# jgrodzki/radix_sort

Hardware: AMD Instinct MI355X
Metric: Gkeys/sec (u64) (higher is better)
Workload: dtype u64

## Files before the change

radix_sort_amd/csrc/rsx_small_kernel.hpp:

```cpp
#pragma once
#include "rsx_device.hpp"
#include "rsx_internal.hpp"

namespace rsx {

struct SmallArgs {
    const void* src;
    void* data;
    uint32_t n;
    uint32_t passes;
    uint32_t rank_atomic;
    uint32_t map_load;
    uint32_t map_store;
    DigitSpec spec[16];
    KeyXform xf;
    const uint32_t* top_tot;
    uint32_t cap;
    uint32_t no_skip;
    uint32_t group_shift;
    uint32_t key_offset, key_bytes;
    uint32_t* hint;
};

struct PassPlan {
    uint32_t first, end;
    uint32_t mask[8];
    uint32_t low[8];
    __device__ __forceinline__ void set_masks(const uint32_t key_offset, const uint32_t key_bytes) {
#pragma unroll
        for (int w = 0; w < 8; ++w) {
            uint32_t m = 0, l = 0;
#pragma unroll
            for (uint32_t b = 0; b < 4; ++b) {
                const uint32_t byte = 4u * (uint32_t)w + b;
                if (byte >= key_offset + first && byte < key_offset + key_bytes) m |= 0xFFu << (8u * b);
                if (byte >= key_offset && byte < key_offset + first) l |= 0xFFu << (8u * b);
            }
            mask[w] = m;
            low[w] = l;
        }
    }
};

#ifndef RSX_MEND_SLACK
#define RSX_MEND_SLACK 6u
#endif
__device__ __forceinline__ uint32_t first_digit_for(const uint32_t m, const uint32_t variable_bits, const uint32_t end) {
    const uint32_t lg = m <= 1u ? 0u : 32u - (uint32_t)__builtin_clz(m - 1u);
    const uint32_t need = 2u * lg > RSX_MEND_SLACK ? 2u * lg - RSX_MEND_SLACK : 0u;
    uint32_t first = variable_bits > need ? (variable_bits - need) >> 3 : 0u;
    if (first + 1u > end) first = end != 0u ? end - 1u : 0u;
    return first;
}

template <int ES>
struct WaveCnt {
    static constexpr bool HALF = false;
    using T = typename std::conditional<HALF, uint16_t, uint32_t>::type;
    static __device__ __forceinline__ void zero(T* my, uint32_t lane) {
        uint32_t* w = reinterpret_cast<uint32_t*>(my);
#pragma unroll
        for (int i = 0; i < (HALF ? 2 : 4); ++i) w[i * WAVE + lane] = 0;
    }
    static __device__ __forceinline__ uint32_t add_rtn(T* my, uint32_t d, uint32_t v) {
        if constexpr (HALF) {
            const uint32_t sh = (d & 1u) * 16u;
            return (atomicAdd(reinterpret_cast<uint32_t*>(my) + (d >> 1), v << sh) >> sh) & 0xFFFFu;
        } else {
            return atomicAdd(&my[d], v);
        }
    }
};
template <int ES, int KPT, int WG>
__host__ __device__ constexpr uint32_t cape() {
    constexpr uint32_t c = rsxh::bucket_cape(ES, KPT, WG);
    return c;
}
template <int ES, int KPT, int WG>
struct LdsTile {
    using C = typename WaveCnt<ES>::T;
    static_assert(sizeof(C) == rsxh::bucket_cnt_bytes(), "host and device agree on the wave counters");
    static constexpr int NWAVE = WG / WAVE;
    __host__ __device__ static constexpr size_t bytes() { return rsxh::lds_tile_bytes(ES, KPT, WG); }
    static __device__ __forceinline__ Elem<ES>* elems(unsigned char* smem) { return reinterpret_cast<Elem<ES>*>(smem); }
    static __device__ __forceinline__ C* cnt(unsigned char* smem) { return reinterpret_cast<C*>(smem + (size_t)cape<ES, KPT, WG>() * ES); }
    static __device__ __forceinline__ uint32_t* misc(unsigned char* smem) { return reinterpret_cast<uint32_t*>(cnt(smem) + NWAVE * RADIX); }
    static __device__ __forceinline__ uint32_t* flag(unsigned char* smem) { return misc(smem) + NWAVE; }
};

struct Slots { uint32_t kp, seg; };
template <int WG>
__device__ __forceinline__ Slots slots_of(const uint32_t n) {
    const uint32_t tid = threadIdx.x, lane = tid & 63u, wave = tid >> 6;
    const uint32_t kp = (n + WG - 1) / WG;
    return Slots{kp, wave * (WAVE * kp) + lane};
}
template <int ES, int KPT, int WG>
__device__ __forceinline__ void local_load(const SmallArgs& a, const Elem<ES>* __restrict__ src, const uint32_t n, Elem<ES> (&e)[KPT]) {
    const Slots sl = slots_of<WG>(n);
    const uint32_t kp = sl.kp, seg = sl.seg;
#pragma unroll
    for (int j = 0; j < KPT; ++j) {
        e[j] = Elem<ES>{};
        if ((uint32_t)j < kp) {
            const uint32_t p = seg + (uint32_t)j * WAVE;
            if (p < n) {
                e[j] = src[p];
                if (a.map_load) key_map<ES, false>(e[j], a.xf);
            }
        }
    }
}

template <int ES, int KPT, int WG>
__device__ __forceinline__ void local_passes(const SmallArgs& a, Elem<ES> (&e)[KPT], const uint32_t n, unsigned char* smem,
                                             const uint32_t first = 0, const uint32_t end = ~0u) {
    const uint32_t stop = end == ~0u ? a.passes : end;
    constexpr int NWAVE = WG / WAVE;
    using E = Elem<ES>;
    using C = WaveCnt<ES>;
    using Tile = LdsTile<ES, KPT, WG>;
    E* s_elems = Tile::elems(smem);
    typename C::T* s_cnt = Tile::cnt(smem);
    uint32_t* s_misc = Tile::misc(smem);
    const uint32_t tid = threadIdx.x, lane = tid & 63u, wave = tid >> 6;
    const Slots sl = slots_of<WG>(n);
    const uint32_t kp = sl.kp, seg = sl.seg;
    typename C::T* my = s_cnt + wave * RADIX;
    for (uint32_t pass = first; pass < stop; ++pass) {
        const DigitSpec spec = a.spec[pass];
        C::zero(my, lane);
        auto digit_of = [&](int j) -> uint32_t {
            return (seg + (uint32_t)j * WAVE >= n) ? 255u : elem_digit<ES, false>(e[j], spec);
        };
        uint32_t rk[KPT];
#pragma unroll
        for (int j = 0; j < KPT; ++j) {
            rk[j] = 0;
            if ((uint32_t)j < kp) {
                const uint32_t d = digit_of(j);
                if (a.rank_atomic) {
                    rk[j] = C::add_rtn(my, d, 1u);
                } else {
                    const uint64_t m = match_digit(d);
                    const uint32_t below = mbcnt64(m);
                    const uint32_t seen = my[d];
                    if (below == 0) (void)C::add_rtn(my, d, (uint32_t)__popcll(m));
                    rk[j] = seen + below;
                }
            }
        }
        __syncthreads();
        uint32_t tcount = 0, incl = 0;
        if (tid < RADIX) {
#pragma unroll
            for (int w = 0; w < NWAVE; ++w) tcount += s_cnt[w * RADIX + tid];
            incl = wave_incl_scan<true>(tcount);
            if (lane == 63) s_misc[wave] = incl;
        }
        __syncthreads();
        if (tid < RADIX) {
            uint32_t run = incl - tcount;
            for (uint32_t w = 0; w < wave; ++w) run += s_misc[w];
#pragma unroll
            for (int w = 0; w < NWAVE; ++w) {
                const uint32_t c = s_cnt[w * RADIX + tid];
                s_cnt[w * RADIX + tid] = (typename C::T)run;
                run += c;
            }
        }
        __syncthreads();
#pragma unroll
        for (int j = 0; j < KPT; ++j)
            if ((uint32_t)j < kp) {
                if constexpr (cape<ES, KPT, WG>() < (uint32_t)WG * KPT) {
                    if (seg + (uint32_t)j * WAVE < n) s_elems[(uint32_t)my[digit_of(j)] + rk[j]] = e[j];
                } else {
                    s_elems[(uint32_t)my[digit_of(j)] + rk[j]] = e[j];
                }
            }
        __syncthreads();
        if (pass + 1 < stop) {
#pragma unroll
            for (int j = 0; j < KPT; ++j)
                if ((uint32_t)j < kp) e[j] = s_elems[seg + (uint32_t)j * WAVE];
        }
    }
}

template <int ES, int KPT, int WG>
__device__ __forceinline__ void local_store(const SmallArgs& a, Elem<ES>* __restrict__ dst, const uint32_t n, unsigned char* smem) {
    const Elem<ES>* s_elems = reinterpret_cast<const Elem<ES>*>(smem);
    for (uint32_t i = threadIdx.x; i < n; i += WG) {
        Elem<ES> x = s_elems[i];
        if (a.map_store) key_map<ES, true>(x, a.xf);
        dst[i] = x;
    }
}

template <int ES, int KPT, int WG>
__device__ __forceinline__ void local_sort(const SmallArgs& a, const Elem<ES>* __restrict__ src, Elem<ES>* __restrict__ dst,
                                           const uint32_t n, unsigned char* smem) {
    Elem<ES> e[KPT];
    local_load<ES, KPT, WG>(a, src, n, e);
    local_passes<ES, KPT, WG>(a, e, n, smem);
    local_store<ES, KPT, WG>(a, dst, n, smem);
}

template <int ES, int KPT, int WG, typename DigitFn>
__device__ __forceinline__ void stream_pass(const SmallArgs& a, const Elem<ES>* __restrict__ src, Elem<ES>* __restrict__ dst, const uint32_t m,
                                            unsigned char* smem, DigitFn digit, const bool map_back, uint32_t& bin_start, uint32_t& bin_count) {
    constexpr int NWAVE = WG / WAVE;
    constexpr uint32_t CH = cape<ES, KPT, WG>();
    using E = Elem<ES>;
    using C = WaveCnt<ES>;
    using Tile = LdsTile<ES, KPT, WG>;
    E* s_elems = Tile::elems(smem);
    typename C::T* s_cnt = Tile::cnt(smem);
    uint32_t* s_misc = Tile::misc(smem);
    uint32_t* s_gbase = s_misc + NWAVE;
    uint32_t* s_dstart = s_gbase + RADIX;
    uint32_t* s_dcount = s_dstart + RADIX;
    const uint32_t tid = threadIdx.x, lane = tid & 63u, wave = tid >> 6;
    typename C::T* my = s_cnt + wave * RADIX;
    if (tid < RADIX) s_gbase[tid] = 0;
    __syncthreads();
    for (uint32_t i = tid; i < m; i += WG) atomicAdd(&s_gbase[digit(src[i])], 1u);
    __syncthreads();
    if (tid < RADIX) {
        const uint32_t c = s_gbase[tid];
        const uint32_t incl = wave_incl_scan<true>(c);
        if (lane == 63) s_misc[wave] = incl;
        s_dcount[tid] = incl - c;
        bin_count = c;
    }
    __syncthreads();
    if (tid < RADIX) {
        uint32_t b = s_dcount[tid];
        for (uint32_t w = 0; w < wave; ++w) b += s_misc[w];
        s_gbase[tid] = b;
        bin_start = b;
    }
    __syncthreads();
    for (uint32_t c0 = 0; c0 < m; c0 += CH) {
        const uint32_t n = m - c0 < CH ? m - c0 : CH;
        const Slots sl = slots_of<WG>(n);
        const uint32_t kp = sl.kp, seg = sl.seg;
        E e[KPT];
#pragma unroll
        for (int j = 0; j < KPT; ++j) {
            e[j] = E{};
            if ((uint32_t)j < kp) {
                const uint32_t p = seg + (uint32_t)j * WAVE;
                if (p < n) e[j] = src[c0 + p];
            }
        }
        C::zero(my, lane);
        auto digit_of = [&](int j) -> uint32_t { return (seg + (uint32_t)j * WAVE >= n) ? 255u : digit(e[j]); };
        uint32_t rk[KPT];
#pragma unroll
        for (int j = 0; j < KPT; ++j) {
            rk[j] = 0;
            if ((uint32_t)j < kp) {
                const uint32_t d = digit_of(j);
                const uint64_t mm = match_digit(d);
                const uint32_t below = mbcnt64(mm);
                const uint32_t seen = my[d];
                if (below == 0) (void)C::add_rtn(my, d, (uint32_t)__popcll(mm));
                rk[j] = seen + below;
            }
        }
        __syncthreads();
        uint32_t tcount = 0, incl = 0;
        if (tid < RADIX) {
#pragma unroll
            for (int w = 0; w < NWAVE; ++w) tcount += s_cnt[w * RADIX + tid];
            incl = wave_incl_scan<true>(tcount);
            if (lane == 63) s_misc[wave] = incl;
        }
        __syncthreads();
        if (tid < RADIX) {
            uint32_t run = incl - tcount;
            for (uint32_t w = 0; w < wave; ++w) run += s_misc[w];
            s_dstart[tid] = run;
            s_dcount[tid] = tid == RADIX - 1 ? tcount - (kp * WG - n) : tcount;
#pragma unroll
            for (int w = 0; w < NWAVE; ++w) {
                const uint32_t c = s_cnt[w * RADIX + tid];
                s_cnt[w * RADIX + tid] = (typename C::T)run;
                run += c;
            }
        }
        __syncthreads();
#pragma unroll
        for (int j = 0; j < KPT; ++j)
            if ((uint32_t)j < kp) {
                if constexpr (cape<ES, KPT, WG>() < (uint32_t)WG * KPT) {
                    if (seg + (uint32_t)j * WAVE < n) s_elems[(uint32_t)my[digit_of(j)] + rk[j]] = e[j];
                } else {
                    s_elems[(uint32_t)my[digit_of(j)] + rk[j]] = e[j];
                }
            }
        __syncthreads();
        for (uint32_t i = tid; i < n; i += WG) {
            E x = s_elems[i];
            const uint32_t d = digit(x);
            const uint32_t pos = s_gbase[d] + (i - s_dstart[d]);
            if (map_back) key_map<ES, true>(x, a.xf);
            dst[pos] = x;
        }
        __syncthreads();
        if (tid < RADIX) s_gbase[tid] += s_dcount[tid];
        __syncthreads();
    }
    __builtin_amdgcn_fence(__ATOMIC_RELEASE, "agent");
    __syncthreads();
    __builtin_amdgcn_fence(__ATOMIC_ACQUIRE, "agent");
}

template <int ES, int KPT, int WG>
__device__ void big_bucket_sort(const SmallArgs& a, Elem<ES>* buf0, Elem<ES>* buf1, const uint32_t m, unsigned char* smem) {
    using E = Elem<ES>;
    E* src = buf0;
    E* dst = buf1;
    for (uint32_t pass = 0; pass < a.passes; ++pass) {
        const DigitSpec spec = a.spec[pass];
        uint32_t bs = 0, bc = 0;
        stream_pass<ES, KPT, WG>(a, src, dst, m, smem, [&](const E& x) { return elem_digit<ES, false>(x, spec); },
                                 pass + 1 == a.passes && a.map_store != 0, bs, bc);
        E* t = src;
        src = dst;
        dst = t;
    }
}

#define RSX_B16_WAVES(WG) ((WG) >= 512 ? 4 : 3)
template <int ES>
__device__ __forceinline__ bool agree(const PassPlan& pp, const Elem<ES>& x, const Elem<ES>& y) {
    uint32_t diff = 0;
#pragma unroll
    for (int w = 0; w < ES / 4; ++w) diff |= (x.w[w] ^ y.w[w]) & pp.mask[w];
    return diff == 0;
}
constexpr uint32_t MEND_LIST = 192;
template <int ES, int KPT, int WG>
__device__ __forceinline__ uint32_t* mend_count(unsigned char* smem) {
    return reinterpret_cast<uint32_t*>(LdsTile<ES, KPT, WG>::cnt(smem));
}
template <int ES, int KPT, int WG>
__device__ __forceinline__ bool local_check(const PassPlan& pp, const uint32_t n, unsigned char* smem, Elem<ES> (&x)[KPT], uint32_t& ties) {
    using E = Elem<ES>;
    const E* s_elems = reinterpret_cast<const E*>(smem);
    ties = 0;
    if (threadIdx.x == 0) *mend_count<ES, KPT, WG>(smem) = 0;
#pragma unroll
    for (int j = 0; j < KPT; ++j) {
        const uint32_t i = (uint32_t)j * WG + threadIdx.x;
        x[j] = E{};
        if (i < n) {
            x[j] = s_elems[i];
            const E p = s_elems[i != 0 ? i - 1 : 0];
            uint32_t diff = 0;
#pragma unroll
            for (int w = 0; w < ES / 4; ++w) diff |= (x[j].w[w] ^ p.w[w]) & pp.mask[w];
            ties |= (diff == 0 && i != 0) ? 1u << j : 0u;
        }
    }
    uint32_t work = 0;
    for (uint32_t t = ties; t != 0; t &= t - 1u) {
        const uint32_t i = (uint32_t)__builtin_ctz(t) * WG + threadIdx.x;
        const E u = s_elems[i], v = s_elems[i - 1];
#pragma unroll
        for (int w = 0; w < ES / 4; ++w) work |= (u.w[w] ^ v.w[w]) & pp.low[w];
    }
    return __syncthreads_or(work != 0 ? 1 : 0) != 0;
}
template <int ES>
struct MendMasks {
    uint32_t hi[ES / 4], lo[ES / 4];
};
template <int ES>
__device__ __forceinline__ uint32_t mend_listed(Elem<ES>* s_elems, uint32_t* s_list, uint32_t* s_flag, const uint32_t n, const uint32_t wg,
                                                        uint32_t ties, const MendMasks<ES> mm) {
    using E = Elem<ES>;
    constexpr uint32_t MAX_RUN = 48;
    auto same = [&](const E& u, const E& v) {
        uint32_t diff = 0;
#pragma unroll
        for (int w = 0; w < ES / 4; ++w) diff |= (u.w[w] ^ v.w[w]) & mm.hi[w];
        return diff == 0;
    };
    auto less = [&](const E& u, const E& v) {
#pragma unroll
        for (int w = ES / 4 - 1; w >= 0; --w) {
            const uint32_t a = u.w[w] & mm.lo[w], b = v.w[w] & mm.lo[w];
            if (a != b) return a < b;
        }
        return false;
    };
    if (threadIdx.x == 0) *s_flag = 0;
    for (uint32_t j = 0; ties != 0; ++j, ties >>= 1) {
        if (!(ties & 1u)) continue;
        const uint32_t i = j * wg + threadIdx.x;
        if (i >= 2 && same(s_elems[i - 1], s_elems[i - 2])) continue;
        const uint32_t k = atomicAdd(&s_list[0], 1u);
        if (k < MEND_LIST) s_list[1 + k] = i - 1;
    }
    __syncthreads();
    const uint32_t heads = s_list[0];
    if (heads > MEND_LIST) return 0u;
    if (threadIdx.x < heads) {
        const uint32_t i = s_list[1 + threadIdx.x];
        uint32_t len = 2;
        while (i + len < n && len <= MAX_RUN && same(s_elems[i + len], s_elems[i])) ++len;
        if (len > MAX_RUN) {
            *s_flag = 1;
        } else {
            for (uint32_t k = 1; k < len; ++k) {
                const E y = s_elems[i + k];
                uint32_t j = k;
                while (j > 0 && less(y, s_elems[i + j - 1])) {
                    s_elems[i + j] = s_elems[i + j - 1];
                    --j;
                }
                s_elems[i + j] = y;
            }
        }
    }
    __syncthreads();
    return *s_flag == 0 ? 1u : 0u;
}
template <int ES, int KPT, int WG>
__device__ __forceinline__ bool local_mend_listed(const uint32_t n, unsigned char* smem, const PassPlan& pp, uint32_t* s_flag, const uint32_t ties) {
    static_assert((WG / WAVE) * RADIX >= MEND_LIST + 1, "the list lives in the wave counters");
    MendMasks<ES> mm;
#pragma unroll
    for (int w = 0; w < ES / 4; ++w) {
        mm.hi[w] = pp.mask[w];
        mm.lo[w] = pp.low[w];
    }
    return mend_listed<ES>(reinterpret_cast<Elem<ES>*>(smem), mend_count<ES, KPT, WG>(smem), s_flag, n, (uint32_t)WG, ties, mm) != 0;
}
template <int ES, int KPT, int WG>
__device__ __forceinline__ void local_store_regs(const SmallArgs& a, Elem<ES>* __restrict__ dst, const uint32_t n, Elem<ES> (&x)[KPT]) {
#pragma unroll
    for (int j = 0; j < KPT; ++j) {
        const uint32_t i = (uint32_t)j * WG + threadIdx.x;
        if (i < n) {
            if (a.map_store) key_map<ES, true>(x[j], a.xf);
            dst[i] = x[j];
        }
    }
}

template <int ES, int KPT, int WG>
__device__ __forceinline__ bool local_mend_pairs(const PassPlan& pp, const uint32_t n, unsigned char* smem) {
    using E = Elem<ES>;
    E* s = reinterpret_cast<E*>(smem);
    uint32_t longer = 0;
#pragma nounroll
    for (uint32_t i = threadIdx.x + 1; i < n; i += WG) {
        const E x = s[i], p = s[i - 1];
        if (!agree<ES>(pp, x, p)) continue;
        bool run = false;
        if (i >= 2) run = agree<ES>(pp, s[i - 2], p);
        if (i + 1 < n) run = run || agree<ES>(pp, s[i + 1], x);
        int order = 0;
#pragma unroll
        for (int w = ES / 4 - 1; w >= 0; --w) {
            const uint32_t u = x.w[w] & pp.low[w], v = p.w[w] & pp.low[w];
            if (order == 0 && u != v) order = u < v ? -1 : 1;
        }
        if (run) {
            longer |= order != 0 ? 1u : 0u;
        } else if (order < 0) {
            s[i - 1] = x;
            s[i] = p;
        }
    }
    return __syncthreads_or((int)longer) != 0;
}

template <int ES, int KPT, int WG, bool PAIRS = false>
__device__ __forceinline__ bool local_finish(const SmallArgs& a, Elem<ES>* __restrict__ dst, const uint32_t n, unsigned char* smem, const PassPlan& pp,
                                             uint32_t* s_flag) {
    Elem<ES> x[KPT];
    uint32_t ties;
    if constexpr (PAIRS) {
        if (!local_mend_pairs<ES, KPT, WG>(pp, n, smem)) {
            const Elem<ES>* s_elems = reinterpret_cast<const Elem<ES>*>(smem);
#pragma unroll
            for (int j = 0; j < KPT; ++j) {
                const uint32_t i = (uint32_t)j * WG + threadIdx.x;
                x[j] = Elem<ES>{};
                if (i < n) x[j] = s_elems[i];
            }
            local_store_regs<ES, KPT, WG>(a, dst, n, x);
            return true;
        }
        (void)local_check<ES, KPT, WG>(pp, n, smem, x, ties);
    } else {
        if (!local_check<ES, KPT, WG>(pp, n, smem, x, ties)) {
            local_store_regs<ES, KPT, WG>(a, dst, n, x);
            return true;
        }
    }
    if (!local_mend_listed<ES, KPT, WG>(n, smem, pp, s_flag, ties)) return false;
    local_store<ES, KPT, WG>(a, dst, n, smem);
    return true;
}

template <int ES, int KPT, int WG, bool PAIRS = false>
__device__ __forceinline__ void local_sort_skip(const SmallArgs& a, const Elem<ES>* __restrict__ src, Elem<ES>* __restrict__ dst, const uint32_t n,
                                                unsigned char* smem, PassPlan& pp, uint32_t* s_flag) {
    using E = Elem<ES>;
    E e[KPT];
    local_load<ES, KPT, WG>(a, src, n, e);
    local_passes<ES, KPT, WG>(a, e, n, smem, pp.first, pp.end);
    if (pp.first == 0) {
        local_store<ES, KPT, WG>(a, dst, n, smem);
    } else if (!local_finish<ES, KPT, WG, PAIRS>(a, dst, n, smem, pp, s_flag)) {
        pp.first = 0;
        const uint32_t kp = (n + WG - 1) / WG, seg = (threadIdx.x >> 6) * (WAVE * kp) + (threadIdx.x & 63u);
#pragma unroll
        for (int j = 0; j < KPT; ++j)
            if ((uint32_t)j < kp) e[j] = reinterpret_cast<const E*>(smem)[seg + (uint32_t)j * WAVE];
        __syncthreads();
        local_passes<ES, KPT, WG>(a, e, n, smem, 0, pp.end);
        local_store<ES, KPT, WG>(a, dst, n, smem);
    }
}

template <int ES, int KPT>
__global__ __launch_bounds__(512) void rsx_small_sort_kernel(const SmallArgs a) {
    extern __shared__ __attribute__((aligned(16))) unsigned char smem[];
    local_sort<ES, KPT, 512>(a, static_cast<const Elem<ES>*>(a.src), static_cast<Elem<ES>*>(a.data), a.n, smem);
}

template <int ES, int KPT, int WG>
__global__ __launch_bounds__(WG) void rsx_bucket_sort_kernel(const SmallArgs a) {
    extern __shared__ __attribute__((aligned(16))) unsigned char smem[];
    uint64_t* s_red = reinterpret_cast<uint64_t*>(smem);
    const uint32_t tid = threadIdx.x, v = blockIdx.x;
    uint64_t c = 0;
    if (tid < RADIX) {
        c = a.top_tot[tid];
        if (tid == v) s_red[4] = c;
        if (v == 0) {
            uint64_t big = c;
#pragma unroll
            for (int o = 32; o > 0; o >>= 1) {
                const uint64_t y = __shfl_xor(big, o);
                big = y > big ? y : big;
            }
            if ((tid & 63u) == 0u) s_red[5 + (tid >> 6)] = big;
        }
        uint64_t below = tid < v ? c : 0ull;
#pragma unroll
        for (int o = 32; o > 0; o >>= 1) below += __shfl_xor(below, o);
        if ((tid & 63u) == 0u) s_red[tid >> 6] = below;
    }
    __syncthreads();
    const uint64_t start = s_red[0] + s_red[1] + s_red[2] + s_red[3];
    const uint64_t count = s_red[4];
    if (v == 0 && tid == 0) {
        uint64_t big = s_red[5];
        for (int w = 1; w < 4; ++w) big = s_red[5 + w] > big ? s_red[5 + w] : big;
        __hip_atomic_store(a.hint, big <= (uint64_t)a.cap / 4 ? 1u : big <= (uint64_t)a.cap ? 3u : 2u, __ATOMIC_RELAXED, __HIP_MEMORY_SCOPE_SYSTEM);
    }
    __syncthreads();
    if (count == 0) return;
    if (count > (uint64_t)cape<ES, KPT, WG>()) {
        big_bucket_sort<ES, KPT, WG>(a, const_cast<Elem<ES>*>(static_cast<const Elem<ES>*>(a.src)) + start,
                                     static_cast<Elem<ES>*>(a.data) + start, (uint32_t)count, smem);
        return;
    }
    if constexpr (ES < 8) {
        local_sort<ES, KPT, WG>(a, static_cast<const Elem<ES>*>(a.src) + start, static_cast<Elem<ES>*>(a.data) + start, (uint32_t)count, smem);
    } else {
        PassPlan pp;
        pp.end = a.passes;
        pp.first = a.no_skip ? 0u : first_digit_for((uint32_t)count, 8u * a.passes, a.passes);
        pp.set_masks(a.key_offset, a.key_bytes);
        uint32_t* s_flag = LdsTile<ES, KPT, WG>::flag(smem);
        local_sort_skip<ES, KPT, WG>(a, static_cast<const Elem<ES>*>(a.src) + start, static_cast<Elem<ES>*>(a.data) + start, (uint32_t)count, smem, pp,
                                     s_flag);
    }
}

template <int ES, int KPT, int WG>
__global__ __launch_bounds__(WG, RSX_B16_WAVES(WG)) void rsx_bucket16_kernel(const SmallArgs a, const uint64_t* __restrict__ starts, void* scratch,
                                                                         const WidePlan* __restrict__ plan, Gate gate,
                                                                         const unsigned char* __restrict__ done, const uint32_t* __restrict__ left) {
    extern __shared__ __attribute__((aligned(16))) unsigned char smem[];
    if (!gate_open(gate)) return;
    using E = Elem<ES>;
    constexpr int NWAVE = WG / WAVE;
    uint32_t* s_flag = LdsTile<ES, KPT, WG>::flag(smem);
    const uint32_t gs = a.group_shift != 0 ? plan->group_shift : 0;
    const bool medium = (plan->verdict & VERDICT_MEDIUM) != 0;
    PassPlan pp;
    pp.end = gs == 0 ? plan->pass_end : plan->group_end;
    if (pp.end == 0) {
        if (a.map_store) {
            const uint64_t n = starts[65536];
            E* data = static_cast<E*>(a.data);
            for (uint64_t i = (uint64_t)blockIdx.x * WG + threadIdx.x; i < n; i += (uint64_t)gridDim.x * WG) {
                E x = data[i];
                key_map<ES, true>(x, a.xf);
                data[i] = x;
            }
        }
        return;
    }
    if (left != nullptr && __builtin_amdgcn_readfirstlane((int)__hip_atomic_load(left, __ATOMIC_RELAXED, __HIP_MEMORY_SCOPE_AGENT)) == 0) return;
    const uint32_t b_lo = plan->window_top - 15u;
    const uint32_t end_sub = pp.end;
    if (gs != 0) pp.end = (b_lo + gs + 7u) / 8u;
    {
        const uint64_t big = (uint64_t)plan->scan_max << gs;
        const uint32_t m = big < (uint64_t)cape<ES, KPT, WG>() ? (uint32_t)big : cape<ES, KPT, WG>();
        pp.first = a.no_skip ? 0u : first_digit_for(m, b_lo + gs, pp.end);
    }
    pp.set_masks(a.key_offset, a.key_bytes);
    for (uint32_t g = blockIdx.x; g < (65536u >> gs); g += gridDim.x) {
        const uint32_t b0 = g << gs;
        const uint64_t gstart = starts[b0];
        const uint64_t gcount = starts[b0 + (1u << gs)] - gstart;
        if (gcount == 0) continue;
        if (done != nullptr && done[g] != 0) continue;
        const bool whole = gs == 0 || gcount <= (uint64_t)cape<ES, KPT, WG>();
        const uint32_t nsub = whole ? 1u : 1u << gs;
        for (uint32_t sub = 0; sub < nsub; ++sub) {
            uint64_t start = gstart, count = gcount;
            if (!whole) {
                start = starts[b0 + sub];
                count = starts[b0 + sub + 1] - start;
            }
            if (count != 0) {
                E* bucket = static_cast<E*>(a.data) + start;
                if (count <= (uint64_t)cape<ES, KPT, WG>()) {
                    const uint32_t first = pp.first, end = pp.end;
                    if (!whole) {
                        pp.first = 0;
                        pp.end = end_sub;
                    }
                    local_sort_skip<ES, KPT, WG, true>(a, bucket, bucket, (uint32_t)count, smem, pp, s_flag);
                    if (!whole) {
                        pp.first = first;
                        pp.end = end;
                    }
                } else if (!medium) {
                    big_bucket_sort<ES, KPT, WG>(a, bucket, static_cast<E*>(scratch) + start, (uint32_t)count, smem);
                }
            }
            __syncthreads();
        }
    }
}

template <int ES, int KPT, int WG>
__global__ __launch_bounds__(WG, RSX_B16_WAVES(WG)) void rsx_bucket16_medium_kernel(const SmallArgs a, const uint64_t* __restrict__ starts, void* scratch,
                                                                                const WidePlan* __restrict__ plan, uint32_t cap256, uint32_t cap512,
                                                                                uint32_t cap1024, Gate gate) {
    extern __shared__ __attribute__((aligned(16))) unsigned char smem[];
    __shared__ uint32_t s_part[2];
    if (!gate_open(gate)) return;
    using E = Elem<ES>;
    constexpr int NWAVE = WG / WAVE;
    constexpr uint32_t CAPE = cape<ES, KPT, WG>();
    uint32_t* s_flag = LdsTile<ES, KPT, WG>::flag(smem);
    const uint32_t tid = threadIdx.x;
    const uint32_t form = plan->verdict & VERDICT_FORM_MASK;
    const uint64_t handled = form == VERDICT_WG256 ? cap256 : form == VERDICT_WG1024 ? cap1024 : cap512;
    const uint32_t end = plan->pass_end;
    if (end == 0) return;
    const uint32_t b_lo = plan->window_top - 15u;
    for (uint32_t b = blockIdx.x; b < 65536u; b += gridDim.x) {
        const uint64_t start = starts[b];
        const uint64_t count = starts[b + 1] - start;
        if (count <= handled) continue;
        E* bucket = static_cast<E*>(a.data) + start;
        E* scr = static_cast<E*>(scratch) + start;
        uint32_t k = 0;
        while (k < 8u && (count >> k) > (uint64_t)CAPE * 6u / 10u) ++k;
        if (k > b_lo) k = b_lo;
        const bool split = !(k == 0 || (count >> k) > (uint64_t)CAPE || count > 0xFFFFFFFFull);
        uint32_t kmask = 0, part_start = 0, part_count = (uint32_t)count;
        PassPlan pp;
        pp.end = end;
        pp.first = 0;
        if (split) {
            DigitSpec sp{};
            const uint32_t ebit = 8u * a.key_offset + b_lo - k;
            sp.word = ebit >> 5;
            sp.shift = ebit & 31u;
            kmask = (1u << k) - 1u;
            part_start = part_count = 0;
            const uint32_t km = kmask;
            stream_pass<ES, KPT, WG>(a, bucket, scr, (uint32_t)count, smem, [&](const E& x) { return elem_digit_any<ES>(x, sp) & km; }, false, part_start,
                                     part_count);
            const uint32_t keep = plan->keep + (k >= 4u ? 1u : 0u);
            pp.first = (end > keep && !a.no_skip) ? end - keep : 0;
            pp.set_masks(a.key_offset, a.key_bytes);
        }
        for (uint32_t j = 0; j <= kmask; ++j) {
            __syncthreads();
            if (tid == j) {
                s_part[0] = part_start;
                s_part[1] = part_count;
            }
            __syncthreads();
            const uint32_t off = s_part[0], cnt = s_part[1];
            if (cnt == 0) continue;
            if (split && cnt <= CAPE) {
                local_sort_skip<ES, KPT, WG>(a, scr + off, bucket + off, cnt, smem, pp, s_flag);
            } else {
                if (split) {
                    for (uint32_t i = tid; i < cnt; i += WG) bucket[off + i] = scr[off + i];
                    __builtin_amdgcn_fence(__ATOMIC_RELEASE, "agent");
                    __syncthreads();
                    __builtin_amdgcn_fence(__ATOMIC_ACQUIRE, "agent");
                }
                big_bucket_sort<ES, KPT, WG>(a, bucket + off, scr + off, cnt, smem);
            }
        }
        __syncthreads();
    }
}

constexpr uint32_t DIRECT_LIMIT = 24;
template <int WG>
__host__ __device__ constexpr uint32_t direct_bits() {
    return WG >= 1024 ? 12u : WG >= 512 ? 11u : 10u;
}
constexpr uint32_t DIRECT_EXTRA_BITS = 1u;
template <int ES>
__device__ __forceinline__ bool key_less(const Elem<ES>& x, const Elem<ES>& y) {
    static_assert(ES == 8 || ES == 16, "key-only elements of 8 and 16 bytes");
    if constexpr (ES == 8) {
        return (((uint64_t)x.w[1] << 32) | x.w[0]) < (((uint64_t)y.w[1] << 32) | y.w[0]);
    } else {
        const uint64_t xh = ((uint64_t)x.w[3] << 32) | x.w[2], yh = ((uint64_t)y.w[3] << 32) | y.w[2];
        const uint64_t xl = ((uint64_t)x.w[1] << 32) | x.w[0], yl = ((uint64_t)y.w[1] << 32) | y.w[0];
        return xh < yh || (xh == yh && xl < yl);
    }
}
__device__ __forceinline__ uint32_t wave_max(uint32_t x) {
    auto step = [](uint32_t v, auto ctrl, auto rows) {
        const uint32_t y = (uint32_t)__builtin_amdgcn_update_dpp(0, (int)v, decltype(ctrl)::value, decltype(rows)::value, 0xf, false);
        return y > v ? y : v;
    };
    x = step(x, std::integral_constant<int, 0x111>{}, std::integral_constant<int, 0xf>{});
    x = step(x, std::integral_constant<int, 0x112>{}, std::integral_constant<int, 0xf>{});
    x = step(x, std::integral_constant<int, 0x114>{}, std::integral_constant<int, 0xf>{});
    x = step(x, std::integral_constant<int, 0x118>{}, std::integral_constant<int, 0xf>{});
    x = step(x, std::integral_constant<int, 0x142>{}, std::integral_constant<int, 0xa>{});
    x = step(x, std::integral_constant<int, 0x143>{}, std::integral_constant<int, 0xc>{});
    return (uint32_t)__builtin_amdgcn_readlane((int)x, 63);
}
template <int ES>
__device__ __forceinline__ void direct_read(const unsigned char* smem, const uint32_t q, Elem<ES> (&y)[16 / ES]) {
    const uint4 v = reinterpret_cast<const uint4*>(smem)[q];
    if constexpr (ES == 8) {
        y[0].w[0] = v.x;
        y[0].w[1] = v.y;
        y[1].w[0] = v.z;
        y[1].w[1] = v.w;
    } else {
        y[0].w[0] = v.x;
        y[0].w[1] = v.y;
        y[0].w[2] = v.z;
        y[0].w[3] = v.w;
    }
}
template <int ES, bool EDGE>
__device__ __forceinline__ void direct_rank(const unsigned char* smem, const uint32_t q, const uint32_t M, const uint32_t n, const Elem<ES> (&x)[16 / ES],
                                            uint32_t (&r)[16 / ES]) {
    constexpr int G = 16 / ES;
    const uint32_t words = (n + G - 1) / G;
#pragma unroll 2
    for (uint32_t m = 1; m <= M; ++m) {
        Elem<ES> lo[G], hi[G];
        uint32_t ql = q - m, qh = q + m;
        bool vl = true, vh = true;
        if constexpr (EDGE) {
            vl = q >= m;
            vh = qh < words;
            ql = vl ? ql : q;
            qh = vh ? qh : q;
        }
        direct_read<ES>(smem, ql, lo);
        direct_read<ES>(smem, qh, hi);
#pragma unroll
        for (int h = 0; h < G; ++h) {
            bool okl = true, okh = true;
            if constexpr (EDGE) {
                okl = vl;
                okh = vh && qh * G + (uint32_t)h < n;
            }
#pragma unroll
            for (int g = 0; g < G; ++g) {
                r[g] -= (okl && key_less<ES>(x[g], lo[h])) ? 1u : 0u;
                r[g] += (okh && key_less<ES>(hi[h], x[g])) ? 1u : 0u;
            }
        }
    }
}

template <int ES, int KPT, int WG>
__global__ __launch_bounds__(WG, RSX_B16_WAVES(WG)) void rsx_bucket16_direct_kernel(const SmallArgs a, const uint64_t* __restrict__ starts,
                                                                                const WidePlan* __restrict__ plan, unsigned char* __restrict__ done,
                                                                                uint32_t* __restrict__ left, Gate gate) {
    extern __shared__ __attribute__((aligned(16))) unsigned char smem[];
    if (!gate_open(gate)) return;
    using E = Elem<ES>;
    constexpr int NWAVE = WG / WAVE;
    constexpr int G = 16 / ES;
    constexpr uint32_t CAPE = cape<ES, KPT, WG>();
    constexpr uint32_t B = direct_bits<WG>(), NB = 1u << B;
    static_assert(NB == (uint32_t)NWAVE * RADIX && NB == 4u * WG && sizeof(typename WaveCnt<ES>::T) == 4, "the counters take the wave counters' place, four to a thread");
    static_assert((CAPE * ES) % 16 == 0, "the counters are read and written as uint4");
    E* s = LdsTile<ES, KPT, WG>::elems(smem);
    uint32_t* s_cnt = LdsTile<ES, KPT, WG>::cnt(smem);
    uint32_t* s_tot = s_cnt + NB + 4;
    const uint32_t tid = threadIdx.x, lane = tid & 63u, wave = tid >> 6;
    constexpr uint32_t BC = B + DIRECT_EXTRA_BITS;
    static_assert(CAPE < (1u << 16), "a count and a start fit a half");
    const uint32_t b_lo = plan->window_top - 15u;
    const uint32_t bd = b_lo < BC ? b_lo : BC;
    const uint32_t dshift = b_lo - bd, dmask = (1u << bd) - 1u;
    const uint32_t dword = dshift >> 5, dsh = dshift & 31u;
    auto digit_of = [&](const E& x) -> uint32_t {
        const uint32_t lo = elem_word<ES>(x, dword);
        const uint32_t hi = elem_word<ES>(x, dword + 1u < (uint32_t)(ES / 4) ? dword + 1u : dword);
        return (uint32_t)(((((uint64_t)hi << 32) | lo) >> dsh)) & dmask;
    };
    auto start_of = [&](const uint32_t d) -> uint32_t {
        return reinterpret_cast<const uint16_t*>(s_cnt)[d];
    };
    auto leave_from = [&](const uint32_t g) -> uint32_t {
        uint32_t mine = 0;
        for (uint32_t b = g + tid * gridDim.x; b < 65536u; b += (uint32_t)WG * gridDim.x) {
            done[b] = 0;
            mine += starts[b + 1] != starts[b] ? 1u : 0u;
        }
        if (tid == 0) s_tot[0] = 0;
        __syncthreads();
        if (mine != 0) atomicAdd(&s_tot[0], mine);
        __syncthreads();
        return s_tot[0];
    };
    uint32_t left_here = 0;
    if (plan->pass_end == 0) {
        if (blockIdx.x < 65536u) left_here = leave_from(blockIdx.x);
        if (tid == 0 && left_here != 0) atomicAdd(left, left_here);
        return;
    }
    for (uint32_t g = blockIdx.x; g < 65536u; g += gridDim.x) {
        const uint64_t start = starts[g];
        const uint64_t count = starts[g + 1] - start;
        if (count == 0 || count > (uint64_t)CAPE) {
            if (tid == 0) done[g] = 0;
            left_here += count != 0 ? 1u : 0u;
            continue;
        }
        const uint32_t n = (uint32_t)count;
        E* bucket = static_cast<E*>(a.data) + start;
        reinterpret_cast<uint4*>(s_cnt)[tid] = uint4{0u, 0u, 0u, 0u};
        E e[KPT];
        constexpr bool LOAD16 = ES == 8 && WG >= 512;
        constexpr int NPAIR = LOAD16 ? KPT / 2 : 0;
        auto pos_of = [&](const int j) -> uint32_t {
            if (j < 2 * NPAIR) return 2u * ((uint32_t)(j >> 1) * WG + tid) + (uint32_t)(j & 1);
            return (uint32_t)j * WG + tid;
        };
        if constexpr (LOAD16) {
            typedef uint32_t v4u __attribute__((ext_vector_type(4)));
            typedef v4u v4u_a8 __attribute__((aligned(8)));
#pragma unroll
            for (int jj = 0; jj < NPAIR; ++jj) {
                const uint32_t i = pos_of(2 * jj);
                e[2 * jj] = E{};
                e[2 * jj + 1] = E{};
                if (i + 1u < n) {
                    const v4u v = *reinterpret_cast<const v4u_a8*>(bucket + i);
                    e[2 * jj].w[0] = v.x, e[2 * jj].w[1] = v.y, e[2 * jj + 1].w[0] = v.z, e[2 * jj + 1].w[1] = v.w;
                }
                if (i + 1u == n) e[2 * jj] = bucket[i];
            }
        }
#pragma unroll
        for (int j = 2 * NPAIR; j < KPT; ++j) {
            const uint32_t i = (uint32_t)j * WG + tid;
            e[j] = E{};
            if (i < n) e[j] = bucket[i];
        }
        __syncthreads();
        uint32_t rk[KPT];
#pragma unroll
        for (int j = 0; j < KPT; ++j) {
            rk[j] = 0;
            if (pos_of(j) < n) {
                const uint32_t d = digit_of(e[j]);
                const uint32_t sh = (d & 1u) << 4;
                rk[j] = (atomicAdd(&s_cnt[d >> 1], 1u << sh) >> sh) & 0xFFFFu;
            }
        }
        __syncthreads();
        const uint4 c = reinterpret_cast<const uint4*>(s_cnt)[tid];
        auto low = [](uint32_t v) { return v & 0xFFFFu; };
        auto larger = [](uint32_t u, uint32_t v) { return u > v ? u : v; };
        const uint32_t p0 = low(c.x) + (c.x >> 16), p1 = low(c.y) + (c.y >> 16), p2 = low(c.z) + (c.z >> 16), p3 = low(c.w) + (c.w >> 16);
        const uint32_t pairs = larger(larger(p0, p1), larger(p2, p3));
        const uint32_t halves = larger(larger(larger(low(c.x), c.x >> 16), larger(low(c.y), c.y >> 16)),
                                       larger(larger(low(c.z), c.z >> 16), larger(low(c.w), c.w >> 16)));
        const uint32_t big = b_lo > B ? pairs : halves;
        const uint32_t sum = p0 + p1 + p2 + p3;
        const uint32_t incl = wave_incl_scan<true>(sum);
        if (lane == 63) s_tot[wave] = incl;
        if (__syncthreads_or(big > DIRECT_LIMIT ? 1 : 0)) {
            left_here += leave_from(g);
            break;
        }
        uint32_t run = incl - sum;
        for (uint32_t w = 0; w < wave; ++w) run += s_tot[w];
        const uint32_t r1 = run + p0, r2 = r1 + p1, r3 = r2 + p2;
        reinterpret_cast<uint4*>(s_cnt)[tid] = uint4{(c.x << 16) + run * 0x10001u, (c.y << 16) + r1 * 0x10001u, (c.z << 16) + r2 * 0x10001u, (c.w << 16) + r3 * 0x10001u};
        if (tid == 0) s_cnt[NB] = n;
        __syncthreads();
#pragma unroll
        for (int j = 0; j < KPT; ++j)
            if (pos_of(j) < n) s[start_of(digit_of(e[j])) + rk[j]] = e[j];
        __syncthreads();
        const uint32_t words = (n + G - 1) / G;
        auto rank_word = [&](const uint32_t q0, const bool live, const uint32_t q, E (&x)[G], uint32_t (&r)[G]) {
            direct_read<ES>(smem, q, x);
            uint32_t need = 0;
#pragma unroll
            for (int h = 0; h < G; ++h) {
                const uint32_t p = q * G + (uint32_t)h;
                r[h] = p;
                if (live && p < n) {
                    const uint32_t d = digit_of(x[h]);
                    const uint32_t below = p - start_of(d), above = start_of(d + 1u) - 1u - p;
                    need = need > below ? need : below;
                    need = need > above ? need : above;
                }
            }
            const uint32_t T = wave_max(need);
            const uint32_t M = (T + G - 1) / G;
            if constexpr (G == 2) {
                const bool both = q * 2u + 1u < n;
                const uint32_t inv = (both && key_less<ES>(x[1], x[0])) ? 1u : 0u;
                r[0] += inv;
                r[1] -= inv;
            }
            if (q0 >= M && q0 + 63u + M < n / G) direct_rank<ES, false>(smem, q, M, n, x, r);
            else direct_rank<ES, true>(smem, q, M, n, x, r);
        };
#pragma nounroll
        for (uint32_t q0 = (uint32_t)__builtin_amdgcn_readfirstlane((int)(tid & ~63u)); q0 < words; q0 += WG) {
            const bool live = q0 + lane < words;
            const uint32_t q = live ? q0 + lane : words - 1u;
            E x[G];
            uint32_t r[G];
            rank_word(q0, live, q, x, r);
#pragma unroll
            for (int h = 0; h < G; ++h)
                if (live && q * G + (uint32_t)h < n) {
                    E y = x[h];
                    if (a.map_store) key_map<ES, true>(y, a.xf);
                    if (r[h] < n) bucket[r[h]] = y;
                }
        }
        if (tid == 0) done[g] = 1;
        __syncthreads();
    }
    if (tid == 0 && left_here != 0) atomicAdd(left, left_here);
}

}
```

Measured before the change: 83.87.

## Prefetch next bucket's keys during ranking and scatter of current bucket

Moves the per-thread key loads into a helper and restructures the bucket loop so the next eligible bucket is looked up early. For 8-byte keys with large workgroups, its first three 16-byte load pairs are issued before the ranking/store phase and the rest after it. This aims to hide global-load latency behind the LDS ranking and global stores of the current bucket. In exchange, the key registers stay live across the rank phase, which raises register pressure and may lower occupancy.

```diff
diff --git a/radix_sort_amd/csrc/rsx_small_kernel.hpp b/radix_sort_amd/csrc/rsx_small_kernel.hpp
--- a/radix_sort_amd/csrc/rsx_small_kernel.hpp
+++ b/radix_sort_amd/csrc/rsx_small_kernel.hpp
@@ -809,6 +809,44 @@
 }
 
 template <int ES, int KPT, int WG>
+struct DirectLoad {
+    using E = Elem<ES>;
+    static constexpr bool LOAD16 = ES == 8 && WG >= 512;
+    static constexpr int NPAIR = LOAD16 ? KPT / 2 : 0;
+    static constexpr bool PIPE = LOAD16;
+    static constexpr int PRE = PIPE ? 3 : 0;
+    static_assert(PRE <= NPAIR, "part 0 is 16-byte words");
+    static __device__ __forceinline__ uint32_t pos_of(const int j, const uint32_t tid) {
+        if (j < 2 * NPAIR) return 2u * ((uint32_t)(j >> 1) * WG + tid) + (uint32_t)(j & 1);
+        return (uint32_t)j * WG + tid;
+    }
+    template <int PART>
+    static __device__ __forceinline__ void load(const E* __restrict__ bucket, const uint32_t n, const uint32_t tid, E (&e)[KPT]) {
+        typedef uint32_t v4u __attribute__((ext_vector_type(4)));
+        typedef v4u v4u_a8 __attribute__((aligned(8)));
+#pragma unroll
+        for (int jj = (PART == 0 ? 0 : PRE); jj < (PART == 0 ? PRE : NPAIR); ++jj) {
+            const uint32_t i = pos_of(2 * jj, tid);
+            e[2 * jj] = E{};
+            e[2 * jj + 1] = E{};
+            if (i + 1u < n) {
+                const v4u v = *reinterpret_cast<const v4u_a8*>(bucket + i);
+                e[2 * jj].w[0] = v.x, e[2 * jj].w[1] = v.y, e[2 * jj + 1].w[0] = v.z, e[2 * jj + 1].w[1] = v.w;
+            }
+            if (i + 1u == n) e[2 * jj] = bucket[i];
+        }
+        if constexpr (PART == 1) {
+#pragma unroll
+            for (int j = 2 * NPAIR; j < KPT; ++j) {
+                const uint32_t i = (uint32_t)j * WG + tid;
+                e[j] = E{};
+                if (i < n) e[j] = bucket[i];
+            }
+        }
+    }
+};
+
+template <int ES, int KPT, int WG>
 __global__ __launch_bounds__(WG, RSX_B16_WAVES(WG)) void rsx_bucket16_direct_kernel(const SmallArgs a, const uint64_t* __restrict__ starts,
                                                                                 const WidePlan* __restrict__ plan, unsigned char* __restrict__ done,
                                                                                 uint32_t* __restrict__ left, Gate gate) {
@@ -857,44 +895,37 @@
         if (tid == 0 && left_here != 0) atomicAdd(left, left_here);
         return;
     }
-    for (uint32_t g = blockIdx.x; g < 65536u; g += gridDim.x) {
-        const uint64_t start = starts[g];
-        const uint64_t count = starts[g + 1] - start;
-        if (count == 0 || count > (uint64_t)CAPE) {
+    using L = DirectLoad<ES, KPT, WG>;
+    auto pos_of = [&](const int j) -> uint32_t { return L::pos_of(j, tid); };
+    auto next_sorted = [&](uint32_t g, E*& bucket, uint32_t& n) -> uint32_t {
+        for (; g < 65536u; g += gridDim.x) {
+            const uint64_t start = starts[g];
+            const uint64_t count = starts[g + 1] - start;
+            if (count != 0 && count <= (uint64_t)CAPE) {
+                bucket = static_cast<E*>(a.data) + start;
+                n = (uint32_t)count;
+                break;
+            }
             if (tid == 0) done[g] = 0;
             left_here += count != 0 ? 1u : 0u;
-            continue;
-        }
-        const uint32_t n = (uint32_t)count;
-        E* bucket = static_cast<E*>(a.data) + start;
+        }
+        return g;
+    };
+    E e[KPT];
+    E* bucket = nullptr;
+    uint32_t n = 0;
+    uint32_t g = next_sorted(blockIdx.x, bucket, n);
+    if constexpr (L::PIPE) {
+        if (g < 65536u) {
+            L::template load<0>(bucket, n, tid, e);
+            L::template load<1>(bucket, n, tid, e);
+        }
+    }
+    while (g < 65536u) {
         reinterpret_cast<uint4*>(s_cnt)[tid] = uint4{0u, 0u, 0u, 0u};
-        E e[KPT];
-        constexpr bool LOAD16 = ES == 8 && WG >= 512;
-        constexpr int NPAIR = LOAD16 ? KPT / 2 : 0;
-        auto pos_of = [&](const int j) -> uint32_t {
-            if (j < 2 * NPAIR) return 2u * ((uint32_t)(j >> 1) * WG + tid) + (uint32_t)(j & 1);
-            return (uint32_t)j * WG + tid;
-        };
-        if constexpr (LOAD16) {
-            typedef uint32_t v4u __attribute__((ext_vector_type(4)));
-            typedef v4u v4u_a8 __attribute__((aligned(8)));
-#pragma unroll
-            for (int jj = 0; jj < NPAIR; ++jj) {
-                const uint32_t i = pos_of(2 * jj);
-                e[2 * jj] = E{};
-                e[2 * jj + 1] = E{};
-                if (i + 1u < n) {
-                    const v4u v = *reinterpret_cast<const v4u_a8*>(bucket + i);
-                    e[2 * jj].w[0] = v.x, e[2 * jj].w[1] = v.y, e[2 * jj + 1].w[0] = v.z, e[2 * jj + 1].w[1] = v.w;
-                }
-                if (i + 1u == n) e[2 * jj] = bucket[i];
-            }
-        }
-#pragma unroll
-        for (int j = 2 * NPAIR; j < KPT; ++j) {
-            const uint32_t i = (uint32_t)j * WG + tid;
-            e[j] = E{};
-            if (i < n) e[j] = bucket[i];
+        if constexpr (!L::PIPE) {
+            L::template load<0>(bucket, n, tid, e);
+            L::template load<1>(bucket, n, tid, e);
         }
         __syncthreads();
         uint32_t rk[KPT];
@@ -933,6 +964,12 @@
         for (int j = 0; j < KPT; ++j)
             if (pos_of(j) < n) s[start_of(digit_of(e[j])) + rk[j]] = e[j];
         __syncthreads();
+        E* next = nullptr;
+        uint32_t n_next = 0;
+        const uint32_t g_next = next_sorted(g + gridDim.x, next, n_next);
+        if constexpr (L::PIPE) {
+            if (g_next < 65536u) L::template load<0>(next, n_next, tid, e);
+        }
         const uint32_t words = (n + G - 1) / G;
         auto rank_word = [&](const uint32_t q0, const bool live, const uint32_t q, E (&x)[G], uint32_t (&r)[G]) {
             direct_read<ES>(smem, q, x);
@@ -974,8 +1011,12 @@
                     if (r[h] < n) bucket[r[h]] = y;
                 }
         }
+        if constexpr (L::PIPE) {
+            if (g_next < 65536u) L::template load<1>(next, n_next, tid, e);
+        }
         if (tid == 0) done[g] = 1;
         __syncthreads();
+        g = g_next, bucket = next, n = n_next;
     }
     if (tid == 0 && left_here != 0) atomicAdd(left, left_here);
 }
```

Measured after the change: 85.84, median of 6. +2.4%, better.
